# hongfz16/Garment4D

Hardware: AMD Instinct MI355X
Metric: point-cloud frames/s (FPS+ball_query+SA-MLP+LBS), B=8 N=8192 (higher is better)
Workload: dtype f32

## Files before the change

### garment4d_amd/csrc/sa_xyz.hip

```cpp
#include <cstdlib>

#include "g4d_common.h"

namespace g4d {

typedef float f32x4 __attribute__((ext_vector_type(4)));

struct SaXyzArgs {
    int n, p, S, logS, pool;
    long long rows;
    const float *xyz, *new_xyz;
    const int *idx;
    const float *W1, *sc1, *sh1;
    int ldw1;
    const float *W2f, *sc2, *sh2;
    const float *W3f, *sc3, *sh3;
    int kst2, kst3;
    float *out;
    int ldo, col0;
};

struct __attribute__((packed, aligned(4))) F3s { float x, y, z; };
__device__ __forceinline__ F3s ld3(const float *base, unsigned elem) {
    return *reinterpret_cast<const F3s *>(reinterpret_cast<const char *>(base) + (elem << 2));
}

__device__ __forceinline__ float pool4_rows_max(float v0, float v1, float v2, float v3) {
    const auto a = __builtin_amdgcn_permlane16_swap(__float_as_uint(v0), __float_as_uint(v1), false, false);
    const auto b = __builtin_amdgcn_permlane16_swap(__float_as_uint(v2), __float_as_uint(v3), false, false);
    const float m01 = fmaxf(__uint_as_float(a[0]), __uint_as_float(a[1]));
    const float m23 = fmaxf(__uint_as_float(b[0]), __uint_as_float(b[1]));
    const auto c = __builtin_amdgcn_permlane32_swap(__float_as_uint(m01), __float_as_uint(m23), false, false);
    return fmaxf(__uint_as_float(c[0]), __uint_as_float(c[1]));
}

template <int C1, int C2, int C3, int LOGS, bool MAXP>
__device__ __forceinline__ void sa_xyz_body(const SaXyzArgs &a, int first, int stride) {
    constexpr int T1 = C1 / 16, T2 = C2 / 16, T3 = C3 / 16;
    constexpr int S = 1 << LOGS;
    static_assert(S == 16 || S == 32, "16 or 32 samples");
    static_assert(T3 == 2 || T3 == 4, "32 or 64 output channels");
    const int lane = threadIdx.x & 63;
    const int fi = lane & 15, fq = lane >> 4;
    float w1f[T1], s1[T1][4], h1s[T1][4];
#pragma unroll
    for (int ks = 0; ks < T1; ++ks) {
        const float w = a.W1[(ks * 16 + fi) * a.ldw1 + min(fq, 2)];
        w1f[ks] = fq < 3 ? w : 0.f;
#pragma unroll
        for (int e = 0; e < 4; ++e) {
            const int c = ks * 16 + fq * 4 + e;
            s1[ks][e] = a.sc1[c]; h1s[ks][e] = a.sh1[c];
        }
    }
    const unsigned cfq = (unsigned)min(fq, 2);
    f32x4 w2[T2][T1], w3[T3][T2];
#pragma unroll
    for (int ct = 0; ct < T2; ++ct)
#pragma unroll
        for (int ks = 0; ks < T1; ++ks) w2[ct][ks] = *reinterpret_cast<const f32x4 *>(a.W2f + ((size_t)(ct * a.kst2 + ks) * 64 + lane) * 4);
#pragma unroll
    for (int ct = 0; ct < T3; ++ct)
#pragma unroll
        for (int ks = 0; ks < T2; ++ks) w3[ct][ks] = *reinterpret_cast<const f32x4 *>(a.W3f + ((size_t)(ct * a.kst3 + ks) * 64 + lane) * 4);
    f32x4 s2[T2], h2s[T2];
#pragma unroll
    for (int ct = 0; ct < T2; ++ct) {
        s2[ct] = *reinterpret_cast<const f32x4 *>(a.sc2 + ct * 16 + fq * 4);
        h2s[ct] = *reinterpret_cast<const f32x4 *>(a.sh2 + ct * 16 + fq * 4);
    }
    float s3[T3], h3s[T3];
#pragma unroll
    for (int ct = 0; ct < T3; ++ct) { s3[ct] = a.sc3[ct * 16 + fi]; h3s[ct] = a.sh3[ct * 16 + fi]; }

    const int rows = (int)a.rows;
    const int npass = (rows + 31) >> 5;
    struct Rows { float px[2], pq[2]; };
    int ivn[2];
    auto load_idx = [&](int pass, int (&v)[2]) {
#pragma unroll
        for (int mt = 0; mt < 2; ++mt) v[mt] = a.idx[min(min(pass, npass - 1) * 32 + mt * 16 + fi, rows - 1)];
    };
    const int nq = (int)(a.rows >> LOGS);
    auto load_rows = [&](int pass, const int (&v)[2], Rows &rw) {
        pass = min(pass, npass - 1);
#pragma unroll
        for (int mt = 0; mt < 2; ++mt) {
            const int qi = __builtin_amdgcn_readfirstlane(min((pass * 32 + mt * 16) >> LOGS, nq - 1));
            const int f = qi / a.p;
            rw.px[mt] = a.xyz[(unsigned)(f * a.n + v[mt]) * 3u + cfq];
            rw.pq[mt] = a.new_xyz[(unsigned)qi * 3u + cfq];
        }
    };
    auto do_pass = [&](int pass, const Rows &cur, Rows &fill, bool alive) {
        load_rows(pass + stride, ivn, fill);
        load_idx(pass + 2 * stride, ivn);
        __builtin_amdgcn_sched_barrier(0);
        const int row0 = pass * 32;
        f32x4 h1[2][T1];
#pragma unroll
        for (int mt = 0; mt < 2; ++mt) {
            const float d = cur.px[mt] - cur.pq[mt];
            const float comp = fq < 3 ? d : 0.f;
#pragma unroll
            for (int ks = 0; ks < T1; ++ks) {
                const f32x4 acc = __builtin_amdgcn_mfma_f32_16x16x4f32(w1f[ks], comp, (f32x4){0.f, 0.f, 0.f, 0.f}, 0, 0, 0);
#pragma unroll
                for (int e = 0; e < 4; ++e) h1[mt][ks][e] = fmaxf(__builtin_fmaf(acc[e], s1[ks][e], h1s[ks][e]), 0.f);
            }
        }
        f32x4 h2[2][T2];
#pragma unroll
        for (int mt = 0; mt < 2; ++mt)
#pragma unroll
            for (int ct = 0; ct < T2; ++ct) h2[mt][ct] = (f32x4){0.f, 0.f, 0.f, 0.f};
#pragma unroll
        for (int ks = 0; ks < T1; ++ks)
#pragma unroll
            for (int e = 0; e < 4; ++e)
#pragma unroll
                for (int mt = 0; mt < 2; ++mt)
#pragma unroll
                    for (int ct = 0; ct < T2; ++ct)
                        h2[mt][ct] = __builtin_amdgcn_mfma_f32_16x16x4f32(w2[ct][ks][e], h1[mt][ks][e], h2[mt][ct], 0, 0, 0);
#pragma unroll
        for (int mt = 0; mt < 2; ++mt)
#pragma unroll
            for (int ct = 0; ct < T2; ++ct)
#pragma unroll
                for (int r = 0; r < 4; ++r) h2[mt][ct][r] = fmaxf(__builtin_fmaf(h2[mt][ct][r], s2[ct][r], h2s[ct][r]), 0.f);
        f32x4 acc[2][T3];
#pragma unroll
        for (int mt = 0; mt < 2; ++mt)
#pragma unroll
            for (int ct = 0; ct < T3; ++ct) acc[mt][ct] = (f32x4){0.f, 0.f, 0.f, 0.f};
#pragma unroll
        for (int ks = 0; ks < T2; ++ks)
#pragma unroll
            for (int e = 0; e < 4; ++e)
#pragma unroll
                for (int mt = 0; mt < 2; ++mt)
#pragma unroll
                    for (int ct = 0; ct < T3; ++ct)
                        acc[mt][ct] = __builtin_amdgcn_mfma_f32_16x16x4f32(h2[mt][ks][e], w3[ct][ks][e], acc[mt][ct], 0, 0, 0);
        if constexpr (MAXP) {
            float v[2][T3];
#pragma unroll
            for (int mt = 0; mt < 2; ++mt)
#pragma unroll
                for (int ct = 0; ct < T3; ++ct) {
                    const float y0 = __builtin_fmaf(acc[mt][ct][0], s3[ct], h3s[ct]), y1 = __builtin_fmaf(acc[mt][ct][1], s3[ct], h3s[ct]),
                                y2 = __builtin_fmaf(acc[mt][ct][2], s3[ct], h3s[ct]), y3 = __builtin_fmaf(acc[mt][ct][3], s3[ct], h3s[ct]);
                    v[mt][ct] = fmaxf(fmaxf(y0, y1), fmaxf(y2, y3));
                }
            if constexpr (S == 32) {
                float x[T3];
#pragma unroll
                for (int ct = 0; ct < T3; ++ct) x[ct] = fmaxf(v[0][ct], v[1][ct]);
                float *o = a.out + (size_t)pass * a.ldo + a.col0;
                if constexpr (T3 == 4) {
                    const float m = fmaxf(pool4_rows_max(x[0], x[1], x[2], x[3]), 0.f);
                    if (alive) o[lane] = m;
                } else {
                    const float m = fmaxf(pool4_rows_max(x[0], x[1], x[0], x[1]), 0.f);
                    if (lane < 32 && alive) o[lane] = m;
                }
            } else {
                if constexpr (T3 == 2) {
                    const float m = fmaxf(pool4_rows_max(v[0][0], v[0][1], v[1][0], v[1][1]), 0.f);
                    const int g = 2 * pass + (lane >> 5);
                    if (g < nq && alive) a.out[(size_t)g * a.ldo + a.col0 + (lane & 31)] = m;
                } else {
#pragma unroll
                    for (int mt = 0; mt < 2; ++mt) {
                        const float m = fmaxf(pool4_rows_max(v[mt][0], v[mt][1], v[mt][2], v[mt][3]), 0.f);
                        if (2 * pass + mt < nq && alive) a.out[(size_t)(2 * pass + mt) * a.ldo + a.col0 + lane] = m;
                    }
                }
            }
        } else {
            constexpr float inv = 1.f / (float)S;
#pragma unroll
            for (int ct = 0; ct < T3; ++ct) {
                float v[2];
#pragma unroll
                for (int mt = 0; mt < 2; ++mt) {
                    float y[4];
#pragma unroll
                    for (int r = 0; r < 4; ++r) y[r] = fmaxf(__builtin_fmaf(acc[mt][ct][r], s3[ct], h3s[ct]), 0.f);
                    float x = (y[0] + y[1]) + (y[2] + y[3]);
                    x = x + lane_xor16(x);
                    x = x + lane_xor32(x);
                    v[mt] = x;
                }
                const int ch = ct * 16 + fi;
                if constexpr (S == 16) {
                    if (lane < 16) {
#pragma unroll
                        for (int mt = 0; mt < 2; ++mt) {
                            const int first_row = row0 + mt * 16;
                            if (first_row < rows && alive) a.out[(size_t)(first_row >> 4) * a.ldo + a.col0 + ch] = v[mt] * inv;
                        }
                    }
                } else {
                    if (lane < 16 && row0 < rows && alive) a.out[(size_t)(row0 >> 5) * a.ldo + a.col0 + ch] = (v[0] + v[1]) * inv;
                }
            }
        }
    };
    int pass = first;
    Rows ra, rb;
    load_idx(pass, ivn);
    load_rows(pass, ivn, ra);
    load_idx(pass + stride, ivn);
    for (; pass < npass; pass += 2 * stride) {
        do_pass(pass, ra, rb, true);
        do_pass(pass + stride, rb, ra, pass + stride < npass);
    }
}

template <int C1, int C2, int C3>
__device__ __forceinline__ void sa_xyz_dispatch(const SaXyzArgs &a, int first, int stride) {
    if (a.pool == 1) {
        if (a.S == 16) sa_xyz_body<C1, C2, C3, 4, true>(a, first, stride);
        else sa_xyz_body<C1, C2, C3, 5, true>(a, first, stride);
    } else {
        if (a.S == 16) sa_xyz_body<C1, C2, C3, 4, false>(a, first, stride);
        else sa_xyz_body<C1, C2, C3, 5, false>(a, first, stride);
    }
}

template <int C1, int C2, int C3>
__global__ void __launch_bounds__(256, 2) sa_xyz_kernel(const SaXyzArgs a) {
    sa_xyz_dispatch<C1, C2, C3>(a, blockIdx.x * 4 + __builtin_amdgcn_readfirstlane(threadIdx.x >> 6), gridDim.x * 4);
}

template <bool MAXP>
__global__ void __launch_bounds__(256, 2) sa_xyz_pair_kernel(const SaXyzArgs a0, const SaXyzArgs a1) {
    const int first = blockIdx.x * 4 + __builtin_amdgcn_readfirstlane(threadIdx.x >> 6), stride = gridDim.x * 4;
    sa_xyz_body<32, 32, 64, 5, MAXP>(a1, first, stride);
    sa_xyz_body<16, 16, 32, 4, MAXP>(a0, first, stride);
}

}

using namespace g4d;

extern "C" int g4d_sa_xyz_mlp3_supported(int c1, int c2, int c3, int nsample) {
    return ((c1 == 16 && c2 == 16 && c3 == 32) || (c1 == 32 && c2 == 32 && c3 == 64)) && (nsample == 16 || nsample == 32);
}

// ... 73 lines not shown
```

### garment4d_amd/csrc/api.hip

```cpp
#include <stdarg.h>
#include <stddef.h>
#include <stdlib.h>
#include <string.h>

#include "mlp_common.h"

namespace g4d {
static thread_local char g_err[512] = "";

void set_error(const char *fmt, ...) {
    va_list ap;
    va_start(ap, fmt);
    vsnprintf(g_err, sizeof(g_err), fmt, ap);
    va_end(ap);
}

static int g_contract = -1;

static int parse_contract(const char *e) {
    if (!e || !*e) return G4D_CONTRACT_NVCC;
    if (!strcmp(e, "0") || !strcmp(e, "off") || !strcmp(e, "none")) return G4D_CONTRACT_OFF;
    if (!strcmp(e, "2") || !strcmp(e, "chain") || !strcmp(e, "inner")) return G4D_CONTRACT_CHAIN;
    return G4D_CONTRACT_NVCC;
}

static thread_local int t_contract = -1;

int distance_contraction() {
    if (t_contract >= 0) return t_contract;
    int m = __atomic_load_n(&g_contract, __ATOMIC_RELAXED);
    if (m < 0) {
        m = parse_contract(getenv("G4D_DIST_CONTRACT"));
        __atomic_store_n(&g_contract, m, __ATOMIC_RELAXED);
    }
    return m;
}
}

namespace g4d {
namespace {
struct Tune { const char *key; long long value; int state; };
Tune g_tune[] = {{"sa_table_persistent", 0, 0}, {"sa_table_min_rows", 0, 0}, {"sa_table_128", 0, 0}, {"sa_table_oversub", 0, 0}, {"sa_table_dedup", 0, 0}, {"fp_table_persistent", 0, 0},
                 {"fp_table_min_rows", 0, 0}, {"gemm_tile", 0, 0}, {"gemm_tile_min_rows", 0, 0}, {"gemm_tile_min_cout", 0, 0}, {"gemm_tile_min_kpad", 0, 0}, {"fp_init_persistent", 0, 0}, {"fp_init_min_rows", 0, 0},
                 {"fp_head_bf16_persistent", 0, 0}, {"fp_head_bf16_min_rows", 0, 0}, {"sa_group_bf16_persistent", 0, 0}, {"sa_group_bf16_min_rows", 0, 0}};
}
struct ThreadTune { long long value; bool set; };
thread_local ThreadTune t_tune[sizeof(g_tune) / sizeof(g_tune[0])] = {};

long long tuning(const char *key, long long dflt) {
    int i = 0;
    for (Tune &t : g_tune) {
        const int slot = i++;
        if (strcmp(t.key, key)) continue;
        if (t_tune[slot].set) return t_tune[slot].value;
        int st = __atomic_load_n(&t.state, __ATOMIC_ACQUIRE);
        if (st == 0) {
            char env[64] = "G4D_";
            size_t n = 4;
            for (const char *c = key; *c && n + 1 < sizeof(env); ++c) env[n++] = (char)((*c >= 'a' && *c <= 'z') ? *c - 32 : *c);
            env[n] = 0;
            const char *e = getenv(env);
            const long long v = e && *e ? atoll(e) : dflt;
            int expect = 0;
            if (__atomic_compare_exchange_n(&t.state, &expect, 3, false, __ATOMIC_ACQ_REL, __ATOMIC_ACQUIRE)) {
                __atomic_store_n(&t.value, v, __ATOMIC_RELAXED);
                expect = 3;
                __atomic_compare_exchange_n(&t.state, &expect, 1, false, __ATOMIC_ACQ_REL, __ATOMIC_ACQUIRE);
                return v;
            }
            st = expect;
            if (st == 3) return v;
        }
        return __atomic_load_n(&t.value, __ATOMIC_RELAXED);
    }
    return dflt;
}
}
// ... 219 lines not shown
```

### garment4d_amd/csrc/fps_bucket.hip

```cpp
#include "g4d_common.h"
#include "ball_grid_build.h"

namespace g4d {

constexpr int kFpsHdr = 2048;

__device__ __forceinline__ unsigned fpsb_rank(int k, int bs, int log2bs) {
    const unsigned c = (unsigned)k & (unsigned)(bs - 1);
    const unsigned q = (unsigned)k >> log2bs;
    const unsigned br = log2bs ? (__builtin_bitreverse32(c) >> (32 - log2bs)) : 0u;
    return (br << 16) | q;
}

__device__ __forceinline__ float fpsb_min(float a, float b) {
    float r;
    asm("v_min_f32 %0, %1, %2" : "=v"(r) : "v"(a), "v"(b));
    return r;
}

template <int W>
__device__ __forceinline__ unsigned long long fpsb_row_max_u64(unsigned long long key) {
#define G4D_STEP(CTRL)                                                                                       \
    {                                                                                                        \
        const unsigned lo = (unsigned)__builtin_amdgcn_update_dpp(0, (int)(unsigned)key, CTRL, 0xf, 0xf, true);        \
        const unsigned hi = (unsigned)__builtin_amdgcn_update_dpp(0, (int)(unsigned)(key >> 32), CTRL, 0xf, 0xf, true); \
        const unsigned long long o = ((unsigned long long)hi << 32) | lo;                                    \
        key = o > key ? o : key;                                                                             \
    }
    G4D_STEP(0x111)
    G4D_STEP(0x112)
    if constexpr (W >= 8) G4D_STEP(0x114)
    if constexpr (W >= 16) G4D_STEP(0x118)
#undef G4D_STEP
    return key;
}

__device__ __forceinline__ float fmax_raw(float a, float b) {
    float r;
// ... 105 lines not shown
#define py(i) pv[P + (i)]
#define pz(i) pv[2 * P + (i)]
#define md(i) pv[3 * P + (i)]
#pragma unroll
    for (int i = 0; i < P; ++i) {
        const int q = (((i / deal) * W + wave) * deal + (i % deal)) * 64 + lane;
        const unsigned long long key = keys[q];
        pk[i] = (key == ~0ull) ? -1 : (int)(unsigned)key;
    }
    __syncthreads();
#pragma unroll
    for (int i = 0; i < P; ++i) {
        const bool ok = pk[i] >= 0;
        const int k = ok ? pk[i] : 0;
        px(i) = ok ? xyz[k * 3 + 0] : 0.f;
        py(i) = ok ? xyz[k * 3 + 1] : 0.f;
        pz(i) = ok ? xyz[k * 3 + 2] : 0.f;
        md(i) = ok ? (temp ? temp[k] : 1e10f) : -2.f;
        if constexpr (SOA) { if (ok) { sx[k] = px(i); sy[k] = py(i); sz[k] = pz(i); } }
    }
    const float x0 = xyz[0], y0 = xyz[1], z0 = xyz[2];
    float blx = INF, bly = INF, blz = INF, bhx = -INF, bhy = -INF, bhz = -INF;
    unsigned rk[P];
#pragma unroll
    for (int i = 0; i < P; ++i) {
        const bool ok = pk[i] >= 0;
        rk[i] = ok ? ((fpsb_rank(pk[i], bs, log2bs) << SB) | (SOA ? 0u : (unsigned)i)) : 0xffffffffu;
        const float a0 = wave_min_f32(ok ? px(i) : INF), a1 = wave_min_f32(ok ? py(i) : INF), a2 = wave_min_f32(ok ? pz(i) : INF);
        const float a3 = wave_max_f32(ok ? px(i) : -INF), a4 = wave_max_f32(ok ? py(i) : -INF), a5 = wave_max_f32(ok ? pz(i) : -INF);
        if ((lane & (P - 1)) == i) { blx = a0; bly = a1; blz = a2; bhx = a3; bhy = a4; bhz = a5; }
    }
    if (t == 0) { spick[0] = 0; slots[0] = 0ull; slots[1] = 0ull; slots[2] = 0ull; }
    if (KMAX > 1 && t == 0) {
        float *res0 = reinterpret_cast<float *>(smem_raw + 1024 + 256);
        res0[0] = x0; res0[1] = y0; res0[2] = z0; res0[3] = INF;
    }
    float *sbox = reinterpret_cast<float *>(smem_raw + kFpsHdr) + (wave * P + (lane & (P - 1))) * 8;
    if constexpr (!SOA) {
        typedef float f32x4b __attribute__((ext_vector_type(4)));
        typedef float f32x2b __attribute__((ext_vector_type(2)));
        if (lane < P) {
            *reinterpret_cast<f32x4b *>(sbox) = (f32x4b){blx, bly, blz, bhx};
            *reinterpret_cast<f32x2b *>(sbox + 4) = (f32x2b){bhy, bhz};
        }
        if (lane < 2) {
            slots[(wave * 2 + lane) * 4] = 0ull;
            reinterpret_cast<float *>(smem_raw)[(wave * 2 + lane) * 8 + 5] = -2.f;
        }
    }
    __syncthreads();

#ifdef G4D_FPS_DEBUG
    unsigned dbg_active = 0;
    long long dbg_t[5] = {0, 0, 0, 0, 0}, dbg_c0 = 0;
#define G4D_STAMP(i) { const long long now_ = clock64(); dbg_t[i] += now_ - dbg_c0; dbg_c0 = now_; }
#else
#define G4D_STAMP(i)
#endif
    if constexpr (KMAX > 1) {
        constexpr int SPP = 64 / P;
        constexpr int KE0 = KMAX;
        constexpr int NK = 2 * W;
        const int KE = min(min(KE0, NK), max(1, kcap));
        static_assert(NK * 32 <= 1024 && 1024 + 256 + KE0 * 16 <= kFpsHdr, "fps multi-pick: the exchange areas must fit the LDS header");
        static_assert(NK <= 64 && KE0 >= 1, "fps multi-pick: key / sample counts must fit a wave");
        unsigned long long *rec = reinterpret_cast<unsigned long long *>(smem_raw);
        unsigned *nstop = reinterpret_cast<unsigned *>(smem_raw + 1024);
        float *res = reinterpret_cast<float *>(smem_raw + 1024 + 256);
        const int ls = lane / P;
        typedef float f32x4 __attribute__((ext_vector_type(4)));
        int ns = 1, j = 1, rpar = 0;
        if (t == 0) { nstop[0] = 0xffu; nstop[1] = 0xffu; }
        float gval = INF;
        unsigned long long rkey = 0ull;
        float rx = x0, ry = y0, rz = z0;
        float rv3 = -2.f;
#ifdef G4D_FPS_DEBUG
        long long dbg_rounds = 0, dbg_stop[4] = {0, 0, 0, 0}, dbg_ph[4] = {0, 0, 0, 0}, dbg_actw = 0, dbg_a[4] = {0, 0, 0, 0}, dbg_pairs = 0, dbg_c1 = 0;
#endif
        while (j < m) {
#ifdef G4D_FPS_DEBUG
            dbg_c0 = clock64(); ++dbg_rounds;
#endif
            if constexpr (!SOA) {
                typedef float f32x4b __attribute__((ext_vector_type(4)));
                typedef float f32x2b __attribute__((ext_vector_type(2)));
                const f32x4b b0 = *reinterpret_cast<const volatile f32x4b *>(sbox);
                const f32x2b b1_ = *reinterpret_cast<const volatile f32x2b *>(sbox + 4);
                blx = b0.x; bly = b0.y; blz = b0.z; bhx = b0.w; bhy = b1_.x; bhz = b1_.y;
            }
            bool swept = false;
            for (int p0 = 0; p0 < ns; p0 += SPP) {
                const f32x4 sv = *reinterpret_cast<const f32x4 *>(&res[min(p0 + ls, KE0 - 1) * 4]);
                const float xs = sv.x, ys = sv.y, zs = sv.z;
                const float gx = fmaxf(fmaxf(blx - xs, xs - bhx), 0.f);
                const float gy = fmaxf(fmaxf(bly - ys, ys - bhy), 0.f);
                const float gz = fmaxf(fmaxf(blz - zs, zs - bhz), 0.f);
                const float dbox = dist2<FM>(gx, gy, gz);
                const unsigned long long active = __builtin_amdgcn_ballot_w64(p0 + ls < ns && dbox < gval);
                if (active == 0ull) continue;
                swept = true;
                const int cnt = min(SPP, ns - p0);
                for (int i = 0; i < cnt; ++i) {
                    const unsigned mi = (unsigned)(active >> (i * P)) & (P >= 32 ? 0xffffffffu : ((1u << (P & 31)) - 1u));
                    if (mi == 0u) continue;
                    const float ax = __int_as_float(__builtin_amdgcn_readlane(__float_as_int(xs), i * P));
                    const float ay = __int_as_float(__builtin_amdgcn_readlane(__float_as_int(ys), i * P));
                    const float az = __int_as_float(__builtin_amdgcn_readlane(__float_as_int(zs), i * P));
#pragma unroll
                    for (int q = 0; q < P; ++q) {
                        if ((mi >> q) & 1u) {
                            const float dx = px(q) - ax, dy = py(q) - ay, dz = pz(q) - az;
                            md(q) = fpsb_min(dist2<FM>(dx, dy, dz), md(q));
                        }
                    }
                }
#ifdef G4D_FPS_DEBUG
                dbg_pairs += __builtin_popcountll(active);
#endif
            }
            if (swept) {
#ifdef G4D_FPS_DEBUG
                { const long long now_ = clock64(); dbg_a[0] += now_ - dbg_c0; dbg_c1 = now_; }
// ... 47 lines not shown
#endif
                const float v2 = lane == h1 ? b2 : b1;
                const unsigned q2 = lane == h1 ? r2 : r1;
                const float c2v = wave_max_f32(v2);
                hit = __builtin_amdgcn_ballot_w64(v2 == c2v);
                unsigned c2r;
                int h2;
                if (__builtin_popcountll(hit) == 1) {
                    h2 = __builtin_ctzll(hit);
                    c2r = (unsigned)__builtin_amdgcn_readlane((int)q2, h2);
                } else {
                    c2r = wave_min_u32(v2 == c2v ? q2 : 0xffffffffu);
                    h2 = __builtin_ctzll(__builtin_amdgcn_ballot_w64(v2 == c2v && q2 == c2r) | (1ull << 63));
                }
                const float v3w = wave_max_f32((lane == h1 || lane == h2) ? b2 : b1);
                if constexpr (SOA) rv3 = v3w;
                {
                    const float cvv = lane == 0 ? c1v : c2v;
                    const unsigned crr = lane == 0 ? c1r : c2r;
                    rkey = (cvv < 0.f || crr == 0xffffffffu) ? 0ull : (((unsigned long long)__float_as_uint(cvv) << 32) | (unsigned)(~crr));
                    if constexpr (SOA) {
                        const unsigned ccls = log2bs ? (__builtin_bitreverse32(crr >> 16) >> (32 - log2bs)) : 0u;
                        const int ci = (rkey && lane < 2) ? (int)(((crr & 0xffffu) << log2bs) | ccls) : 0;
                        rx = sx[ci]; ry = sy[ci]; rz = sz[ci];
                    } else {
                        const int s1 = (int)(c1r & (unsigned)(P - 1)), s2 = (int)(c2r & (unsigned)(P - 1));
                        const float ax1 = pv[s1], ay1 = pv[P + s1], az1 = pv[2 * P + s1];
                        const float ax2 = pv[s2], ay2 = pv[P + s2], az2 = pv[2 * P + s2];
                        const float bx1 = __int_as_float(__builtin_amdgcn_readlane(__float_as_int(ax1), h1)), bx2 = __int_as_float(__builtin_amdgcn_readlane(__float_as_int(ax2), h2));
                        const float by1 = __int_as_float(__builtin_amdgcn_readlane(__float_as_int(ay1), h1)), by2 = __int_as_float(__builtin_amdgcn_readlane(__float_as_int(ay2), h2));
                        const float bz1 = __int_as_float(__builtin_amdgcn_readlane(__float_as_int(az1), h1)), bz2 = __int_as_float(__builtin_amdgcn_readlane(__float_as_int(az2), h2));
                        rx = lane == 0 ? bx1 : bx2; ry = lane == 0 ? by1 : by2; rz = lane == 0 ? bz1 : bz2;
                        if (lane < 2) {
                            typedef unsigned long long u64x2 __attribute__((ext_vector_type(2)));
                            *reinterpret_cast<u64x2 *>(&rec[(wave * 2 + lane) * 4]) = (u64x2){rkey, ((unsigned long long)__float_as_uint(ry) << 32) | __float_as_uint(rx)};
                            typedef float f32x2b __attribute__((ext_vector_type(2)));
                            *reinterpret_cast<f32x2b *>(reinterpret_cast<float *>(rec) + (wave * 2 + lane) * 8 + 4) = (f32x2b){rz, v3w};
                        }
                    }
                }
#ifdef G4D_FPS_DEBUG
                { const long long now_ = clock64(); dbg_a[3] += now_ - dbg_c1; dbg_c1 = now_; }
#endif
            }
#ifdef G4D_FPS_DEBUG
            { const long long now_ = clock64(); dbg_ph[0] += now_ - dbg_c0; dbg_c0 = now_; dbg_actw += swept; }
#endif
            if (SOA && lane < 2) {
                typedef unsigned long long u64x2 __attribute__((ext_vector_type(2)));
                typedef float f32x2b __attribute__((ext_vector_type(2)));
                *reinterpret_cast<u64x2 *>(&rec[(wave * 2 + lane) * 4]) = (u64x2){rkey, ((unsigned long long)__float_as_uint(ry) << 32) | __float_as_uint(rx)};
                *reinterpret_cast<f32x2b *>(reinterpret_cast<float *>(rec) + (wave * 2 + lane) * 8 + 4) = (f32x2b){rz, rv3};
            }
            __syncthreads();
#ifdef G4D_FPS_DEBUG
            { const long long now_ = clock64(); dbg_ph[1] += now_ - dbg_c0; dbg_c0 = now_; }
#endif
            {
                const int c = lane >> 5, jj = lane & 31;
                const float *recf = reinterpret_cast<const float *>(rec);
                const unsigned long long kj = jj < NK ? rec[jj * 4] : 0ull;
                const float jx = recf[jj * 8 + 2], jy = recf[jj * 8 + 3], jz = recf[jj * 8 + 4];
                const int me = wave * 2 + c;
                const unsigned long long km = rec[me * 4];
                const float mx = recf[me * 8 + 2], my = recf[me * 8 + 3], mz = recf[me * 8 + 4];
                const float mv = __uint_as_float((unsigned)(km >> 32));
                const bool gt = kj > km;
                const bool aff = gt && !(dist2<FM>(mx - jx, my - jy, mz - jz) >= mv);
                const unsigned long long gtm = __builtin_amdgcn_ballot_w64(gt), afm = __builtin_amdgcn_ballot_w64(aff);
                const unsigned gth = c ? (unsigned)(gtm >> 32) : (unsigned)gtm, afh = c ? (unsigned)(afm >> 32) : (unsigned)afm;
                const int rank = __builtin_popcount(gth);
                const float v3j = recf[(jj >> 1) * 16 + 5];
                const unsigned both = gth & (gth >> 1) & 0x55555555u;
                const bool hid = ((both >> (jj & ~1)) & 1u) != 0u && !(mv > v3j);
                const unsigned long long hdm = __builtin_amdgcn_ballot_w64(hid);
                const unsigned hdh = c ? (unsigned)(hdm >> 32) : (unsigned)hdm;
                const bool zero = !(mv > 0.f);
                const bool bad = km == 0ull || afh != 0u || hdh != 0u || (zero && rank > 0);
                const bool after = zero;
                if (jj == 0) {
                    atomicMin(&nstop[rpar], bad ? (unsigned)rank : (after ? (unsigned)rank + 1u : 0xffu));
                    if (rank < KE) {
                        const unsigned crk = (~(unsigned)km) >> SB;
                        const unsigned ccls = log2bs ? (__builtin_bitreverse32(crk >> 16) >> (32 - log2bs)) : 0u;
                        *reinterpret_cast<f32x4 *>(&res[rank * 4]) = (f32x4){mx, my, mz, mv};
                        if (j + rank < m) spick[j + rank] = km ? (int)(((crk & 0xffffu) << log2bs) | ccls) : 0;
                    }
                }
                if (t == 0) nstop[rpar ^ 1] = 0xffu;
            }
            __syncthreads();
            {
                int n = __builtin_amdgcn_readfirstlane((int)nstop[rpar]);
                n = max(1, min(min(n, KE), m - j));
                gval = res[(n - 1) * 4 + 3];
                ns = n;
            }
            rpar ^= 1;
            j += ns;
#ifdef G4D_FPS_DEBUG
            { const long long now_ = clock64(); dbg_ph[2] += now_ - dbg_c0; dbg_c0 = now_; }
#endif
        }
        if (temp && ns > 1) {
            if constexpr (!SOA) {
                blx = sbox[0]; bly = sbox[1]; blz = sbox[2]; bhx = sbox[3]; bhy = sbox[4]; bhz = sbox[5];
            }
            for (int p0 = 0; p0 < ns - 1; p0 += SPP) {
                const f32x4 sv = *reinterpret_cast<const f32x4 *>(&res[min(p0 + ls, KE0 - 1) * 4]);
                const float xs = sv.x, ys = sv.y, zs = sv.z;
                const float gx = fmaxf(fmaxf(blx - xs, xs - bhx), 0.f);
                const float gy = fmaxf(fmaxf(bly - ys, ys - bhy), 0.f);
                const float gz = fmaxf(fmaxf(blz - zs, zs - bhz), 0.f);
                const unsigned long long active = __builtin_amdgcn_ballot_w64(p0 + ls < ns - 1 && dist2<FM>(gx, gy, gz) < INF);
                const int cnt = min(SPP, ns - 1 - p0);
                for (int i = 0; i < cnt; ++i) {
                    const unsigned mi = (unsigned)(active >> (i * P)) & (P >= 32 ? 0xffffffffu : ((1u << (P & 31)) - 1u));
                    const float ax = __int_as_float(__builtin_amdgcn_readlane(__float_as_int(xs), i * P));
                    const float ay = __int_as_float(__builtin_amdgcn_readlane(__float_as_int(ys), i * P));
                    const float az = __int_as_float(__builtin_amdgcn_readlane(__float_as_int(zs), i * P));
#pragma unroll
                    for (int q = 0; q < P; ++q)
                        if ((mi >> q) & 1u) md(q) = fpsb_min(dist2<FM>(px(q) - ax, py(q) - ay, pz(q) - az), md(q));
// ... 100 lines not shown
    }
#undef px
#undef py
#undef pz
#undef md
#ifdef G4D_FPS_DEBUG
    __syncthreads();
    if (lane == 0 && temp) atomicAdd(&temp[0], (float)dbg_active);
    if (lane == 0 && temp && (wave == 0 || wave == 5) && cloud == 0)
        for (int q = 0; q < 4; ++q) temp[1 + (wave ? 4 : 0) + q] = (float)dbg_t[q];
#endif
}

template <int W, int P, int FM, int KMAX>
__global__ void __launch_bounds__(64 * W) fps_bucket_kernel(int n, int m, int bs, int log2bs, int deal, int pick_off, const float *__restrict__ xyz_all,
                                                           float *__restrict__ temp_all, int *__restrict__ idx_all, float *__restrict__ nx_all) {
    fps_bucket_body<W, P, FM, KMAX, true>(n, m, bs, log2bs, deal, pick_off, xyz_all, temp_all, idx_all, nx_all, blockIdx.x);
}

template <int W, int P, int FM, int KMAX>
__global__ void __launch_bounds__(64 * W) __attribute__((amdgpu_waves_per_eu(7, 8)))
fps_bucket_reg_kernel(int n, int m, int bs, int log2bs, int deal, int pick_off, const float *__restrict__ xyz_all, float *__restrict__ temp_all,
                      int *__restrict__ idx_all, float *__restrict__ nx_all) {
    fps_bucket_body<W, P, FM, KMAX, false>(n, m, bs, log2bs, deal, pick_off, xyz_all, temp_all, idx_all, nx_all, blockIdx.x);
}

constexpr int kFpsPicks = 16;
static int fps_multi() {
    static const int k = getenv("G4D_FPS_MULTI") ? atoi(getenv("G4D_FPS_MULTI")) : 8;
    return k > 1 ? 8 : 1;
}
static bool fps_soa(int b) {
    static const int k = getenv("G4D_FPS_SOA") ? atoi(getenv("G4D_FPS_SOA")) : -1;
    return k < 0 ? b < 32 : k != 0;
}
static int fps_kcap() {
    static const int k = getenv("G4D_FPS_KCAP") ? atoi(getenv("G4D_FPS_KCAP")) : kFpsPicks;
    return k < 1 ? 1 : (k > 64 ? 64 : k);
}

template <int FM, int KMAX>
__global__ void __launch_bounds__(1024) fps_bucket_grid_kernel(int b, int n, int m, int bs, int log2bs, int deal, int pick_off,
                                                              const float *__restrict__ xyz_all, int *__restrict__ idx_all, float *__restrict__ nx_all,
                                                              int cmax, float cell_req, unsigned char *__restrict__ ws_all, size_t ws_stride) {
    if ((int)blockIdx.x < b) fps_bucket_body<16, 8, FM, KMAX, true>(n, m, bs, log2bs, deal, pick_off, xyz_all, nullptr, idx_all, nx_all, blockIdx.x);
    else ball_grid_build_body(n, cmax, cmax, cell_req, xyz_all, ws_all, ws_stride, (int)blockIdx.x - b);
}

template <int FM, int KMAX>
__global__ void __launch_bounds__(1024) __attribute__((amdgpu_waves_per_eu(7, 8)))
fps_bucket_grid_reg_kernel(int b, int n, int m, int bs, int log2bs, int deal, int pick_off, const float *__restrict__ xyz_all, int *__restrict__ idx_all,
                           float *__restrict__ nx_all, int cmax, float cell_req, unsigned char *__restrict__ ws_all, size_t ws_stride) {
    if ((int)blockIdx.x < b) fps_bucket_body<16, 8, FM, KMAX, false>(n, m, bs, log2bs, deal, pick_off, xyz_all, nullptr, idx_all, nx_all, blockIdx.x);
    else ball_grid_build_body(n, cmax, cmax, cell_req, xyz_all, ws_all, ws_stride, (int)blockIdx.x - b);
}

template <int W, int P, int FM>
static int launch_bucket_fm(int b, int n, int m, int bs, int log2bs, const float *xyz, float *temp, int *idx, float *nx, hipStream_t s) {
    const size_t npad = (size_t)64 * W * P;
    const bool multi = fps_multi() > 1;
    const bool soa = !multi || fps_soa(b) || W != 16;
    const size_t body = (!soa || npad * 8 > (size_t)n * 12) ? npad * 8 : (size_t)n * 12;
    const size_t pick_off = (kFpsHdr + body + 15) & ~(size_t)15;
    const size_t lds = pick_off + (size_t)m * 4;
    if (lds > 160 * 1024 - 1024) return -1;
    auto kern = multi ? fps_bucket_kernel<W, P, FM, kFpsPicks> : fps_bucket_kernel<W, P, FM, 1>;
    if constexpr (W == 16) { if (!soa) kern = fps_bucket_reg_kernel<W, P, FM, kFpsPicks>; }
    static unsigned long long attr_done[3] = {0, 0, 0};
    if (const int rc = ensure_dynamic_lds(reinterpret_cast<const void *>(kern), 160 * 1024 - 1024, attr_done[multi ? (soa ? 1 : 2) : 0], "g4d_fps_f32(bucketed)")) return rc;
    static const int deal_env = getenv("G4D_FPS_DEAL") ? atoi(getenv("G4D_FPS_DEAL")) : 0;
    const int deal = (deal_env >= 1 && deal_env <= P && P % deal_env == 0) ? deal_env : P;
// ... 50 lines not shown
```

### garment4d_amd/tuning.py

```python
import contextlib
import contextvars
import dataclasses
import os
from typing import Mapping, Tuple


def _env_flag(name, default):
    return os.environ.get(name, "1" if default else "0") != "0"


def _env_int(name, default):
    return int(os.environ.get(name, str(default)))


NATIVE_KEYS = ("sa_table_persistent", "sa_table_min_rows", "sa_table_128", "sa_table_oversub", "sa_table_dedup", "fp_table_persistent", "fp_table_min_rows", "gemm_tile",
               "gemm_tile_min_rows", "gemm_tile_min_cout", "gemm_tile_min_kpad", "fp_init_persistent", "fp_init_min_rows",
               "fp_head_bf16_persistent", "fp_head_bf16_min_rows", "sa_group_bf16_persistent", "sa_group_bf16_min_rows")


@dataclasses.dataclass(frozen=True)
class Tuning:
    use_wave: bool = True
    use_stack: bool = True
    use_chain: bool = True
    stream_gemm: bool = True
    bf16_min_rows: int = 0
    overlap_sampling: bool = False
    lanes_sort: bool = False
    coherent_lanes: bool = False
    grid_min_n: int = 4096
    fps_pair: bool = True
    bq_multi: bool = True
    search_multi: bool = True
    three_nn_grid_min_m: int = 4096
    nn_cells: bool = True
    nn_multi: bool = True
    nn_prune: bool = True
    sa_xyz_pair: bool = True
    use_sa_xyz: bool = True
    sa_xyz_table: bool = True
    sa_table: bool = True
    fp_wide_fused: bool = False
    fp_cells: bool = True
    fp_table: bool = True
    fp_gemm_bf16: bool = True
    fp_gemm_bf16_min_rows: int = 8192
    fp_wide_table: bool = True
    dropin_fused: bool = True
    dropin_whole_model: bool = True
    use_pe_kernel: bool = True
# ... 78 lines not shown
```

Measured before the change: 52610.

## Skip duplicate ball-query tiles and hoist BN affine past max-pool

For max-pooled S=32 groups, each wave uses a ballot to check whether the second 16-row tile holds only copies of the first index (ball-query padding). If so, it computes just one MFMA tile and skips the duplicated work. When every BN3 scale is positive, the affine is applied after the max instead of per element. Pass order is rotated across waves with a stride permutation to spread skip-heavy work. This adds branching, doubles code instantiations, and can raise register pressure.

```diff
diff --git a/garment4d_amd/csrc/sa_xyz.hip b/garment4d_amd/csrc/sa_xyz.hip
--- a/garment4d_amd/csrc/sa_xyz.hip
+++ b/garment4d_amd/csrc/sa_xyz.hip
@@ -34,6 +34,8 @@
     return fmaxf(__uint_as_float(c[0]), __uint_as_float(c[1]));
 }
 
+template <int N> struct Tag { static constexpr int value = N; };
+
 template <int C1, int C2, int C3, int LOGS, bool MAXP>
 __device__ __forceinline__ void sa_xyz_body(const SaXyzArgs &a, int first, int stride) {
     constexpr int T1 = C1 / 16, T2 = C2 / 16, T3 = C3 / 16;
@@ -72,6 +74,15 @@
     float s3[T3], h3s[T3];
 #pragma unroll
     for (int ct = 0; ct < T3; ++ct) { s3[ct] = a.sc3[ct * 16 + fi]; h3s[ct] = a.sh3[ct * 16 + fi]; }
+    float s3o = 0.f, h3o = 0.f;
+    bool hoist = false;
+    if constexpr (MAXP) {
+        s3o = a.sc3[lane & (C3 - 1)]; h3o = a.sh3[lane & (C3 - 1)];
+        bool pos = true;
+#pragma unroll
+        for (int ct = 0; ct < T3; ++ct) pos = pos && __float_as_uint(s3[ct]) - 1u < 0x7f800000u;
+        hoist = __builtin_amdgcn_ballot_w64(!pos) == 0ull;
+    }
 
     const int rows = (int)a.rows;
     const int npass = (rows + 31) >> 5;
@@ -92,14 +103,16 @@
             rw.pq[mt] = a.new_xyz[(unsigned)qi * 3u + cfq];
         }
     };
-    auto do_pass = [&](int pass, const Rows &cur, Rows &fill, bool alive) {
-        load_rows(pass + stride, ivn, fill);
-        load_idx(pass + 2 * stride, ivn);
-        __builtin_amdgcn_sched_barrier(0);
+    constexpr bool SKIP = MAXP && S == 32;
+    auto second_tile_alive = [&](const int (&v)[2]) { return __builtin_amdgcn_ballot_w64(v[1] != __builtin_amdgcn_readlane(v[0], 0)) != 0ull; };
+    bool two_cur = true;
+    auto compute = [&](auto nt_tag, auto hoist_tag, int pass, const Rows &cur, bool alive) {
+        constexpr int NT = decltype(nt_tag)::value;
+        constexpr bool HOIST = decltype(hoist_tag)::value != 0;
         const int row0 = pass * 32;
         f32x4 h1[2][T1];
 #pragma unroll
-        for (int mt = 0; mt < 2; ++mt) {
+        for (int mt = 0; mt < NT; ++mt) {
             const float d = cur.px[mt] - cur.pq[mt];
             const float comp = fq < 3 ? d : 0.f;
 #pragma unroll
@@ -111,7 +124,7 @@
         }
         f32x4 h2[2][T2];
 #pragma unroll
-        for (int mt = 0; mt < 2; ++mt)
+        for (int mt = 0; mt < NT; ++mt)
 #pragma unroll
             for (int ct = 0; ct < T2; ++ct) h2[mt][ct] = (f32x4){0.f, 0.f, 0.f, 0.f};
 #pragma unroll
@@ -119,19 +132,19 @@
 #pragma unroll
             for (int e = 0; e < 4; ++e)
 #pragma unroll
-                for (int mt = 0; mt < 2; ++mt)
+                for (int mt = 0; mt < NT; ++mt)
 #pragma unroll
                     for (int ct = 0; ct < T2; ++ct)
                         h2[mt][ct] = __builtin_amdgcn_mfma_f32_16x16x4f32(w2[ct][ks][e], h1[mt][ks][e], h2[mt][ct], 0, 0, 0);
 #pragma unroll
-        for (int mt = 0; mt < 2; ++mt)
+        for (int mt = 0; mt < NT; ++mt)
 #pragma unroll
             for (int ct = 0; ct < T2; ++ct)
 #pragma unroll
                 for (int r = 0; r < 4; ++r) h2[mt][ct][r] = fmaxf(__builtin_fmaf(h2[mt][ct][r], s2[ct][r], h2s[ct][r]), 0.f);
         f32x4 acc[2][T3];
 #pragma unroll
-        for (int mt = 0; mt < 2; ++mt)
+        for (int mt = 0; mt < NT; ++mt)
 #pragma unroll
             for (int ct = 0; ct < T3; ++ct) acc[mt][ct] = (f32x4){0.f, 0.f, 0.f, 0.f};
 #pragma unroll
@@ -139,41 +152,49 @@
 #pragma unroll
             for (int e = 0; e < 4; ++e)
 #pragma unroll
-                for (int mt = 0; mt < 2; ++mt)
+                for (int mt = 0; mt < NT; ++mt)
 #pragma unroll
                     for (int ct = 0; ct < T3; ++ct)
                         acc[mt][ct] = __builtin_amdgcn_mfma_f32_16x16x4f32(h2[mt][ks][e], w3[ct][ks][e], acc[mt][ct], 0, 0, 0);
         if constexpr (MAXP) {
             float v[2][T3];
-#pragma unroll
-            for (int mt = 0; mt < 2; ++mt)
-#pragma unroll
-                for (int ct = 0; ct < T3; ++ct) {
-                    const float y0 = __builtin_fmaf(acc[mt][ct][0], s3[ct], h3s[ct]), y1 = __builtin_fmaf(acc[mt][ct][1], s3[ct], h3s[ct]),
-                                y2 = __builtin_fmaf(acc[mt][ct][2], s3[ct], h3s[ct]), y3 = __builtin_fmaf(acc[mt][ct][3], s3[ct], h3s[ct]);
-                    v[mt][ct] = fmaxf(fmaxf(y0, y1), fmaxf(y2, y3));
-                }
+            if constexpr (HOIST) {
+#pragma unroll
+                for (int mt = 0; mt < NT; ++mt)
+#pragma unroll
+                    for (int ct = 0; ct < T3; ++ct) v[mt][ct] = fmaxf(fmaxf(fmaxf(acc[mt][ct][0], acc[mt][ct][1]), acc[mt][ct][2]), acc[mt][ct][3]);
+            } else {
+#pragma unroll
+                for (int mt = 0; mt < NT; ++mt)
+#pragma unroll
+                    for (int ct = 0; ct < T3; ++ct) {
+                        const float y0 = __builtin_fmaf(acc[mt][ct][0], s3[ct], h3s[ct]), y1 = __builtin_fmaf(acc[mt][ct][1], s3[ct], h3s[ct]),
+                                    y2 = __builtin_fmaf(acc[mt][ct][2], s3[ct], h3s[ct]), y3 = __builtin_fmaf(acc[mt][ct][3], s3[ct], h3s[ct]);
+                        v[mt][ct] = fmaxf(fmaxf(y0, y1), fmaxf(y2, y3));
+                    }
+            }
+            auto finish = [&](float m) { return fmaxf(HOIST ? __builtin_fmaf(m, s3o, h3o) : m, 0.f); };
             if constexpr (S == 32) {
                 float x[T3];
 #pragma unroll
-                for (int ct = 0; ct < T3; ++ct) x[ct] = fmaxf(v[0][ct], v[1][ct]);
+                for (int ct = 0; ct < T3; ++ct) x[ct] = NT == 2 ? fmaxf(v[0][ct], v[1][ct]) : v[0][ct];
                 float *o = a.out + (size_t)pass * a.ldo + a.col0;
                 if constexpr (T3 == 4) {
-                    const float m = fmaxf(pool4_rows_max(x[0], x[1], x[2], x[3]), 0.f);
+                    const float m = finish(pool4_rows_max(x[0], x[1], x[2], x[3]));
                     if (alive) o[lane] = m;
                 } else {
-                    const float m = fmaxf(pool4_rows_max(x[0], x[1], x[0], x[1]), 0.f);
+                    const float m = finish(pool4_rows_max(x[0], x[1], x[0], x[1]));
                     if (lane < 32 && alive) o[lane] = m;
                 }
             } else {
                 if constexpr (T3 == 2) {
-                    const float m = fmaxf(pool4_rows_max(v[0][0], v[0][1], v[1][0], v[1][1]), 0.f);
+                    const float m = finish(pool4_rows_max(v[0][0], v[0][1], v[1][0], v[1][1]));
                     const int g = 2 * pass + (lane >> 5);
                     if (g < nq && alive) a.out[(size_t)g * a.ldo + a.col0 + (lane & 31)] = m;
                 } else {
 #pragma unroll
-                    for (int mt = 0; mt < 2; ++mt) {
-                        const float m = fmaxf(pool4_rows_max(v[mt][0], v[mt][1], v[mt][2], v[mt][3]), 0.f);
+                    for (int mt = 0; mt < NT; ++mt) {
+                        const float m = finish(pool4_rows_max(v[mt][0], v[mt][1], v[mt][2], v[mt][3]));
                         if (2 * pass + mt < nq && alive) a.out[(size_t)(2 * pass + mt) * a.ldo + a.col0 + lane] = m;
                     }
                 }
@@ -208,15 +229,45 @@
             }
         }
     };
-    int pass = first;
-    Rows ra, rb;
-    load_idx(pass, ivn);
-    load_rows(pass, ivn, ra);
-    load_idx(pass + stride, ivn);
-    for (; pass < npass; pass += 2 * stride) {
-        do_pass(pass, ra, rb, true);
-        do_pass(pass + stride, rb, ra, pass + stride < npass);
-    }
+    auto do_pass = [&](auto hoist_tag, int pass, int pass1, int pass2, const Rows &cur, Rows &fill, bool alive) {
+        load_rows(pass1, ivn, fill);
+        bool two_nxt = true;
+        if constexpr (SKIP) two_nxt = second_tile_alive(ivn);
+        load_idx(pass2, ivn);
+        __builtin_amdgcn_sched_barrier(0);
+        if constexpr (SKIP) {
+            if (two_cur) compute(Tag<2>{}, hoist_tag, pass, cur, alive);
+            else compute(Tag<1>{}, hoist_tag, pass, cur, alive);
+            two_cur = two_nxt;
+        } else {
+            compute(Tag<2>{}, hoist_tag, pass, cur, alive);
+        }
+    };
+    constexpr int kRot = 1189;
+    auto run = [&](auto hoist_tag) {
+        const int rot = SKIP ? kRot % stride : 0;
+        int base = 0, slot = first;
+        auto next_pass = [&] {
+            base += stride;
+            slot += rot;
+            if (slot >= stride) slot -= stride;
+            return base + slot;
+        };
+        int p0 = first, p1 = next_pass(), p2 = next_pass();
+        Rows ra, rb;
+        load_idx(p0, ivn);
+        if constexpr (SKIP) two_cur = second_tile_alive(ivn);
+        load_rows(p0, ivn, ra);
+        load_idx(p1, ivn);
+        while (p0 < npass) {
+            do_pass(hoist_tag, p0, p1, p2, ra, rb, true);
+            const int p3 = next_pass();
+            do_pass(hoist_tag, p1, p2, p3, rb, ra, p1 < npass);
+            p0 = p2; p1 = p3; p2 = next_pass();
+        }
+    };
+    if (hoist) run(Tag<1>{});
+    else run(Tag<0>{});
 }
 
 template <int C1, int C2, int C3>
```

New measurement: 52430, median of 2. No clear change (-0.3%).

## Split FPS exchange records into SoA LDS arrays and skip unneeded conflict checks

Applied to the files above, without the earlier changes.

The per-wave pick records in LDS change from an interleaved 32-byte struct to separate key, xy and zv arrays. The conflict-check phase now computes the distance and hidden-pair ballots only when some lane's rank can fall below the pick cap. The bounding-box reload moves before the barrier so it overlaps the wait. FPS kcap and the SoA threshold become thread-tunable knobs, with the NK limit tightened to 32.

```diff
diff --git a/garment4d_amd/csrc/api.hip b/garment4d_amd/csrc/api.hip
--- a/garment4d_amd/csrc/api.hip
+++ b/garment4d_amd/csrc/api.hip
@@ -42,7 +42,8 @@
 struct Tune { const char *key; long long value; int state; };
 Tune g_tune[] = {{"sa_table_persistent", 0, 0}, {"sa_table_min_rows", 0, 0}, {"sa_table_128", 0, 0}, {"sa_table_oversub", 0, 0}, {"sa_table_dedup", 0, 0}, {"fp_table_persistent", 0, 0},
                  {"fp_table_min_rows", 0, 0}, {"gemm_tile", 0, 0}, {"gemm_tile_min_rows", 0, 0}, {"gemm_tile_min_cout", 0, 0}, {"gemm_tile_min_kpad", 0, 0}, {"fp_init_persistent", 0, 0}, {"fp_init_min_rows", 0, 0},
-                 {"fp_head_bf16_persistent", 0, 0}, {"fp_head_bf16_min_rows", 0, 0}, {"sa_group_bf16_persistent", 0, 0}, {"sa_group_bf16_min_rows", 0, 0}};
+                 {"fp_head_bf16_persistent", 0, 0}, {"fp_head_bf16_min_rows", 0, 0}, {"sa_group_bf16_persistent", 0, 0}, {"sa_group_bf16_min_rows", 0, 0},
+                 {"fps_reg_min_clouds", 0, 0}, {"fps_kcap", 0, 0}};
 }
 struct ThreadTune { long long value; bool set; };
 thread_local ThreadTune t_tune[sizeof(g_tune) / sizeof(g_tune[0])] = {};
diff --git a/garment4d_amd/csrc/fps_bucket.hip b/garment4d_amd/csrc/fps_bucket.hip
--- a/garment4d_amd/csrc/fps_bucket.hip
+++ b/garment4d_amd/csrc/fps_bucket.hip
@@ -4,6 +4,9 @@
 namespace g4d {
 
 constexpr int kFpsHdr = 2048;
+constexpr int kFpsRecKey = 0, kFpsRecXY = 256, kFpsRecZV = 512;
+constexpr int kFpsStop = 1024;
+constexpr int kFpsRes = 1280;
 
 __device__ __forceinline__ unsigned fpsb_rank(int k, int bs, int log2bs) {
     const unsigned c = (unsigned)k & (unsigned)(bs - 1);
@@ -175,7 +178,7 @@
     }
     if (t == 0) { spick[0] = 0; slots[0] = 0ull; slots[1] = 0ull; slots[2] = 0ull; }
     if (KMAX > 1 && t == 0) {
-        float *res0 = reinterpret_cast<float *>(smem_raw + 1024 + 256);
+        float *res0 = reinterpret_cast<float *>(smem_raw + kFpsRes);
         res0[0] = x0; res0[1] = y0; res0[2] = z0; res0[3] = INF;
     }
     float *sbox = reinterpret_cast<float *>(smem_raw + kFpsHdr) + (wave * P + (lane & (P - 1))) * 8;
@@ -187,8 +190,8 @@
             *reinterpret_cast<f32x2b *>(sbox + 4) = (f32x2b){bhy, bhz};
         }
         if (lane < 2) {
-            slots[(wave * 2 + lane) * 4] = 0ull;
-            reinterpret_cast<float *>(smem_raw)[(wave * 2 + lane) * 8 + 5] = -2.f;
+            reinterpret_cast<unsigned long long *>(smem_raw + kFpsRecKey)[wave * 2 + lane] = 0ull;
+            reinterpret_cast<float *>(smem_raw + kFpsRecZV)[(wave * 2 + lane) * 2 + 1] = -2.f;
         }
     }
     __syncthreads();
@@ -205,16 +208,32 @@
         constexpr int KE0 = KMAX;
         constexpr int NK = 2 * W;
         const int KE = min(min(KE0, NK), max(1, kcap));
-        static_assert(NK * 32 <= 1024 && 1024 + 256 + KE0 * 16 <= kFpsHdr, "fps multi-pick: the exchange areas must fit the LDS header");
-        static_assert(NK <= 64 && KE0 >= 1, "fps multi-pick: key / sample counts must fit a wave");
-        unsigned long long *rec = reinterpret_cast<unsigned long long *>(smem_raw);
-        unsigned *nstop = reinterpret_cast<unsigned *>(smem_raw + 1024);
-        float *res = reinterpret_cast<float *>(smem_raw + 1024 + 256);
+        static_assert(NK <= 32 && kFpsRecKey + 32 * 8 <= kFpsRecXY && kFpsRecXY + 32 * 8 <= kFpsRecZV && kFpsRecZV + 32 * 8 <= kFpsStop && kFpsStop + 8 <= kFpsRes &&
+                          kFpsRes + KE0 * 16 <= kFpsHdr, "fps multi-pick: the exchange areas must fit the LDS header");
+        static_assert(KE0 >= 1, "fps multi-pick: key / sample counts must fit a wave");
+        typedef float f32x2 __attribute__((ext_vector_type(2)));
+        unsigned long long *rkeys = reinterpret_cast<unsigned long long *>(smem_raw + kFpsRecKey);
+        f32x2 *rxy = reinterpret_cast<f32x2 *>(smem_raw + kFpsRecXY);
+        f32x2 *rzv = reinterpret_cast<f32x2 *>(smem_raw + kFpsRecZV);
+        unsigned *nstop = reinterpret_cast<unsigned *>(smem_raw + kFpsStop);
+        float *res = reinterpret_cast<float *>(smem_raw + kFpsRes);
         const int ls = lane / P;
         typedef float f32x4 __attribute__((ext_vector_type(4)));
         int ns = 1, j = 1, rpar = 0;
         if (t == 0) { nstop[0] = 0xffu; nstop[1] = 0xffu; }
         float gval = INF;
+        auto load_boxes = [&]() {
+            if constexpr (!SOA) {
+                typedef float f32x4b __attribute__((ext_vector_type(4)));
+                typedef float f32x2b __attribute__((ext_vector_type(2)));
+                typedef const volatile __attribute__((address_space(3))) f32x4b *lds4;
+                typedef const volatile __attribute__((address_space(3))) f32x2b *lds2;
+                const f32x4b b0 = *(lds4)(sbox);
+                const f32x2b b1_ = *(lds2)(sbox + 4);
+                blx = b0.x; bly = b0.y; blz = b0.z; bhx = b0.w; bhy = b1_.x; bhz = b1_.y;
+            }
+        };
+        load_boxes();
         unsigned long long rkey = 0ull;
         float rx = x0, ry = y0, rz = z0;
         float rv3 = -2.f;
@@ -225,13 +244,6 @@
 #ifdef G4D_FPS_DEBUG
             dbg_c0 = clock64(); ++dbg_rounds;
 #endif
-            if constexpr (!SOA) {
-                typedef float f32x4b __attribute__((ext_vector_type(4)));
-                typedef float f32x2b __attribute__((ext_vector_type(2)));
-                const f32x4b b0 = *reinterpret_cast<const volatile f32x4b *>(sbox);
-                const f32x2b b1_ = *reinterpret_cast<const volatile f32x2b *>(sbox + 4);
-                blx = b0.x; bly = b0.y; blz = b0.z; bhx = b0.w; bhy = b1_.x; bhz = b1_.y;
-            }
             bool swept = false;
             for (int p0 = 0; p0 < ns; p0 += SPP) {
                 const f32x4 sv = *reinterpret_cast<const f32x4 *>(&res[min(p0 + ls, KE0 - 1) * 4]);
@@ -345,10 +357,9 @@
                         const float bz1 = __int_as_float(__builtin_amdgcn_readlane(__float_as_int(az1), h1)), bz2 = __int_as_float(__builtin_amdgcn_readlane(__float_as_int(az2), h2));
                         rx = lane == 0 ? bx1 : bx2; ry = lane == 0 ? by1 : by2; rz = lane == 0 ? bz1 : bz2;
                         if (lane < 2) {
-                            typedef unsigned long long u64x2 __attribute__((ext_vector_type(2)));
-                            *reinterpret_cast<u64x2 *>(&rec[(wave * 2 + lane) * 4]) = (u64x2){rkey, ((unsigned long long)__float_as_uint(ry) << 32) | __float_as_uint(rx)};
-                            typedef float f32x2b __attribute__((ext_vector_type(2)));
-                            *reinterpret_cast<f32x2b *>(reinterpret_cast<float *>(rec) + (wave * 2 + lane) * 8 + 4) = (f32x2b){rz, v3w};
+                            rkeys[wave * 2 + lane] = rkey;
+                            rxy[wave * 2 + lane] = (f32x2){rx, ry};
+                            rzv[wave * 2 + lane] = (f32x2){rz, v3w};
                         }
                     }
                 }
@@ -360,10 +371,9 @@
             { const long long now_ = clock64(); dbg_ph[0] += now_ - dbg_c0; dbg_c0 = now_; dbg_actw += swept; }
 #endif
             if (SOA && lane < 2) {
-                typedef unsigned long long u64x2 __attribute__((ext_vector_type(2)));
-                typedef float f32x2b __attribute__((ext_vector_type(2)));
-                *reinterpret_cast<u64x2 *>(&rec[(wave * 2 + lane) * 4]) = (u64x2){rkey, ((unsigned long long)__float_as_uint(ry) << 32) | __float_as_uint(rx)};
-                *reinterpret_cast<f32x2b *>(reinterpret_cast<float *>(rec) + (wave * 2 + lane) * 8 + 4) = (f32x2b){rz, rv3};
+                rkeys[wave * 2 + lane] = rkey;
+                rxy[wave * 2 + lane] = (f32x2){rx, ry};
+                rzv[wave * 2 + lane] = (f32x2){rz, rv3};
             }
             __syncthreads();
 #ifdef G4D_FPS_DEBUG
@@ -371,37 +381,43 @@
 #endif
             {
                 const int c = lane >> 5, jj = lane & 31;
-                const float *recf = reinterpret_cast<const float *>(rec);
-                const unsigned long long kj = jj < NK ? rec[jj * 4] : 0ull;
-                const float jx = recf[jj * 8 + 2], jy = recf[jj * 8 + 3], jz = recf[jj * 8 + 4];
+                const unsigned long long kj = jj < NK ? rkeys[jj] : 0ull;
                 const int me = wave * 2 + c;
-                const unsigned long long km = rec[me * 4];
-                const float mx = recf[me * 8 + 2], my = recf[me * 8 + 3], mz = recf[me * 8 + 4];
-                const float mv = __uint_as_float((unsigned)(km >> 32));
+                const unsigned long long km = rkeys[me];
+                f32x2 jxy = rxy[jj], jzv = rzv[jj], mxy = rxy[me], mzv = rzv[me];
+                asm volatile("" : "+v"(jxy), "+v"(jzv), "+v"(mxy), "+v"(mzv));
                 const bool gt = kj > km;
-                const bool aff = gt && !(dist2<FM>(mx - jx, my - jy, mz - jz) >= mv);
-                const unsigned long long gtm = __builtin_amdgcn_ballot_w64(gt), afm = __builtin_amdgcn_ballot_w64(aff);
-                const unsigned gth = c ? (unsigned)(gtm >> 32) : (unsigned)gtm, afh = c ? (unsigned)(afm >> 32) : (unsigned)afm;
+                const unsigned long long gtm = __builtin_amdgcn_ballot_w64(gt);
+                const unsigned gth = c ? (unsigned)(gtm >> 32) : (unsigned)gtm;
                 const int rank = __builtin_popcount(gth);
-                const float v3j = recf[(jj >> 1) * 16 + 5];
-                const unsigned both = gth & (gth >> 1) & 0x55555555u;
-                const bool hid = ((both >> (jj & ~1)) & 1u) != 0u && !(mv > v3j);
-                const unsigned long long hdm = __builtin_amdgcn_ballot_w64(hid);
-                const unsigned hdh = c ? (unsigned)(hdm >> 32) : (unsigned)hdm;
-                const bool zero = !(mv > 0.f);
-                const bool bad = km == 0ull || afh != 0u || hdh != 0u || (zero && rank > 0);
-                const bool after = zero;
-                if (jj == 0) {
-                    atomicMin(&nstop[rpar], bad ? (unsigned)rank : (after ? (unsigned)rank + 1u : 0xffu));
-                    if (rank < KE) {
-                        const unsigned crk = (~(unsigned)km) >> SB;
-                        const unsigned ccls = log2bs ? (__builtin_bitreverse32(crk >> 16) >> (32 - log2bs)) : 0u;
-                        *reinterpret_cast<f32x4 *>(&res[rank * 4]) = (f32x4){mx, my, mz, mv};
-                        if (j + rank < m) spick[j + rank] = km ? (int)(((crk & 0xffffu) << log2bs) | ccls) : 0;
+                if (min(__builtin_popcount((unsigned)gtm), __builtin_popcount((unsigned)(gtm >> 32))) < KE) {
+                    const float jx = jxy.x, jy = jxy.y, jz = jzv.x;
+                    const float mx = mxy.x, my = mxy.y, mz = mzv.x;
+                    const float mv = __uint_as_float((unsigned)(km >> 32));
+                    const bool aff = gt && !(dist2<FM>(mx - jx, my - jy, mz - jz) >= mv);
+                    const unsigned long long afm = __builtin_amdgcn_ballot_w64(aff);
+                    const unsigned afh = c ? (unsigned)(afm >> 32) : (unsigned)afm;
+                    const float v3j = jzv.y;
+                    const unsigned both = gth & (gth >> 1) & 0x55555555u;
+                    const bool hid = ((both >> (jj & ~1)) & 1u) != 0u && !(mv > v3j);
+                    const unsigned long long hdm = __builtin_amdgcn_ballot_w64(hid);
+                    const unsigned hdh = c ? (unsigned)(hdm >> 32) : (unsigned)hdm;
+                    const bool zero = !(mv > 0.f);
+                    const bool bad = km == 0ull || afh != 0u || hdh != 0u || (zero && rank > 0);
+                    const bool after = zero;
+                    if (jj == 0) {
+                        atomicMin(&nstop[rpar], bad ? (unsigned)rank : (after ? (unsigned)rank + 1u : 0xffu));
+                        if (rank < KE) {
+                            const unsigned crk = (~(unsigned)km) >> SB;
+                            const unsigned ccls = log2bs ? (__builtin_bitreverse32(crk >> 16) >> (32 - log2bs)) : 0u;
+                            *reinterpret_cast<f32x4 *>(&res[rank * 4]) = (f32x4){mx, my, mz, mv};
+                            if (j + rank < m) spick[j + rank] = km ? (int)(((crk & 0xffffu) << log2bs) | ccls) : 0;
+                        }
                     }
                 }
                 if (t == 0) nstop[rpar ^ 1] = 0xffu;
             }
+            load_boxes();
             __syncthreads();
             {
                 int n = __builtin_amdgcn_readfirstlane((int)nstop[rpar]);
@@ -568,11 +584,11 @@
 }
 static bool fps_soa(int b) {
     static const int k = getenv("G4D_FPS_SOA") ? atoi(getenv("G4D_FPS_SOA")) : -1;
-    return k < 0 ? b < 32 : k != 0;
+    return k < 0 ? (long long)b < tuning("fps_reg_min_clouds", 32) : k != 0;
 }
 static int fps_kcap() {
-    static const int k = getenv("G4D_FPS_KCAP") ? atoi(getenv("G4D_FPS_KCAP")) : kFpsPicks;
-    return k < 1 ? 1 : (k > 64 ? 64 : k);
+    const long long k = tuning("fps_kcap", kFpsPicks);
+    return k < 1 ? 1 : (k > 64 ? 64 : (int)k);
 }
 
 template <int FM, int KMAX>
diff --git a/garment4d_amd/tuning.py b/garment4d_amd/tuning.py
--- a/garment4d_amd/tuning.py
+++ b/garment4d_amd/tuning.py
@@ -15,7 +15,8 @@
 
 NATIVE_KEYS = ("sa_table_persistent", "sa_table_min_rows", "sa_table_128", "sa_table_oversub", "sa_table_dedup", "fp_table_persistent", "fp_table_min_rows", "gemm_tile",
                "gemm_tile_min_rows", "gemm_tile_min_cout", "gemm_tile_min_kpad", "fp_init_persistent", "fp_init_min_rows",
-               "fp_head_bf16_persistent", "fp_head_bf16_min_rows", "sa_group_bf16_persistent", "sa_group_bf16_min_rows")
+               "fp_head_bf16_persistent", "fp_head_bf16_min_rows", "sa_group_bf16_persistent", "sa_group_bf16_min_rows",
+               "fps_reg_min_clouds", "fps_kcap")
 
 
 @dataclasses.dataclass(frozen=True)
```

After: 52280 before, 53470 after, median of 4. No clear change (+2.3%).
